# hyf015/egocentric-gaze-prediction

Measured on AMD Instinct MI355X. Metric: SP+AT train frames/sec/node (224x224, bs32/GPU), higher is better.
Workload: dtype f32 (every convolution -- forward, data gradient, weight gradient -- as f16 split-half MFMA, abs-max scaled operands, THREE products per MAC: 22 significant bits on both operands of every product; fp32 accumulate; everything else exact f32)

## Files before the change

### egocentric-gaze-prediction_amd/_lib.py

```python
from __future__ import annotations

import ctypes
import os
from ctypes import c_char_p, c_double, c_float, c_int, c_long, c_size_t, c_void_p

_HERE = os.path.dirname(os.path.abspath(__file__))
LIB_PATH = os.environ.get("EGAZE_HIP_LIB") or os.path.join(_HERE, "csrc", "libegaze_hip.so")

P = c_void_p
S = c_void_p

SIGNATURES = {
    "egz_version": (c_char_p, []),
    "egz_last_error": (c_char_p, []),
    "egz_mfma_probe": (c_int, [P, P, c_int, c_int, S]),
    "egz_u8_center_of_mass": (c_int, [P, c_int, c_int, c_int, P, P, P, S]),
    "egz_bilinear_up": (c_int, [P, P, c_int, c_int, c_int, c_int, c_int, c_long, S]),
    "egz_pack_w3x3_elems": (c_size_t, [c_int, c_int, c_int]),
    "egz_pack_w3x3_ups_fwd": (c_int, [P, P, c_int, c_int, S]),
    "egz_pack_w3x3_ups_dgrad": (c_int, [P, P, c_int, c_int, S]),
    "egz_conv3x3_ups_dgrad": (c_int, [P, P, P, c_int, c_int, c_int, c_int, c_int, c_int, S]),
    "egz_pack_w3x3_fwd": (c_int, [P, P, c_int, c_int, S]),
    "egz_pack_w3x3_dgrad": (c_int, [P, P, c_int, c_int, S]),
    "egz_conv3x3_stat_rows": (c_int, [c_int, c_int, c_int, c_int, c_int]),
# ... 66 lines not shown
    "egz_mse_bwd": (c_int, [P, P, P, P, c_long, c_int, S]),
    "egz_mse_fwd_grad": (c_int, [P, P, P, P, c_long, c_int, P, c_int, P, S]),
    "egz_gemm": (c_int, [P, P, P, P, c_int, c_int, c_int, c_long, c_long, c_long, c_long, c_long, c_int, S]),
    "egz_gemm_batched": (c_int, [P, P, P, c_int, c_int, c_int, c_int, c_long, c_long, c_long, c_long, c_long, c_int, S]),
    "egz_lstm_cell_fwd": (c_int, [P, P, P, P, P, c_int, c_int, S]),
    "egz_lstm_cell_bwd": (c_int, [P, P, P, P, P, P, P, c_int, c_int, S]),
    "egz_lstm_wave_fwd": (c_int, [P, P, P, P, P, P, P, P, P, P, P, c_int, c_int, c_int, c_int, S]),
    "egz_lstm_persist_sync_words": (c_int, []),
    "egz_lstm_persist_fwd": (c_int, [P, P, P, P, P, P, P, P, P, P, P, P, P, c_int, c_int, c_int, c_int, S]),
    "egz_lstm_persist_bwd": (c_int, [P, P, P, P, P, P, P, P, P, P, P, P, P, c_int, c_int, c_int, c_int, S]),
    "egz_lstm_wave_bwd": (c_int, [P, P, P, P, P, P, P, P, P, P, P, P, c_int, c_int, c_int, c_int, S]),
    "egz_lstm_b1_ws_bytes": (c_size_t, [c_int, c_int, c_int, c_int]),
    "egz_lstm_b1_fwd": (c_int, [P, c_int, P, P, P, P, P, P, P, P, c_int, c_int, c_int, S]),
    "egz_lstm_b1_bwd": (c_int, [P, P, c_int, P, P, P, P, P, P, P, P, P, P, c_int, c_int, c_int, P, c_size_t, S]),
    "egz_tanh_fwd": (c_int, [P, P, c_long, S]),
    "egz_tanh_bwd": (c_int, [P, P, P, c_long, S]),
    "egz_add": (c_int, [P, P, P, c_long, S]),
    "egz_cat2_planes": (c_int, [P, P, P, c_int, c_long, S]),
    "egz_u8_normalize": (c_int, [P, P, c_long, c_long, c_int, P, P, S]),
    "egz_crop_mean": (c_int, [P, P, P, c_int, c_int, c_int, c_int, c_int, c_int, S]),
    "egz_window_mean": (c_int, [P, P, P, c_int, c_int, c_int, c_int, S]),
    "egz_pixel_weighted_sum": (c_int, [P, P, P, c_int, c_int, c_int, S]),
    "egz_weighted_minmax": (c_int, [P, P, P, c_int, c_int, c_int, S]),
    "egz_aae_auc": (c_int, [P, P, c_int, c_int, c_int, P, c_int, c_double, P, S]),
    "egz_gaze_gt_maps": (c_int, [P, c_int, c_int, c_int, P, c_int, P, P, P, c_int, P, P, P, c_int, c_int, c_int, c_int,
                                 P, P, P, S]),
    "egz_resize_linear_u8": (c_int, [P, c_int, c_int, c_int, c_int, c_int, c_int, c_int, P, P, P, P, P, S]),
    "egz_heatmap_overlay": (c_int, [P, c_int, c_int, c_int, P, P, c_int, c_int, c_int, P, P, P, P, P, P, S]),
    "egz_cell_argmax_u8": (c_int, [P, c_int, c_int, c_int, c_int, P, S]),
    "egz_jpeg_decode_ws_bytes": (c_size_t, [c_int, c_int, c_int, c_int]),
    "egz_jpeg_decode": (c_int, [P, c_long, P, P, P, c_int, c_int, c_int, P, c_long, P, P, c_size_t, c_int, c_int, S]),
    "egz_adam_step": (c_int, [P, P, P, P, c_long, c_double, c_double, c_double, c_double, c_int, c_double, P, S]),
    "egz_adam_step_dev": (c_int, [P, P, P, P, c_long, c_double, c_double, c_double, c_double, P, c_double, P, S]),
}


class EgazeHipError(RuntimeError):
    """Raised when a C-ABI entry point returns a non-zero code (mirrors the reference's convention of
    plain Python exceptions: utils.generalException / RuntimeError, SURVEY.md 8b)."""


def _load():
    if not os.path.exists(LIB_PATH):
        raise ImportError(
            f"{LIB_PATH} is missing: the HIP extension is mandatory (no CPU fallback). "
            "Build it with `python __graft_entry__.py` or `csrc/build.sh`.")
    import torch
    lib = ctypes.CDLL(LIB_PATH)
    for name, (res, args) in SIGNATURES.items():
        try:
            fn = getattr(lib, name)
        except AttributeError as e:
            raise ImportError(f"{LIB_PATH} does not export {name}; rebuild the extension") from e
        fn.restype = res
        fn.argtypes = args
    return lib


LIB = _load()


def check(rc: int, what: str = ""):
    if rc != 0:
        msg = LIB.egz_last_error().decode(errors="replace")
        raise EgazeHipError(f"{what or 'egaze-hip'} failed (code {rc}): {msg}")

# ... 4 lines not shown
```

### egocentric-gaze-prediction_amd/csrc/adam.hip

```cpp
#include "egz_common.h"

namespace {
__global__ __launch_bounds__(256) void adam_kernel(float* __restrict__ p, const float* __restrict__ g, float* __restrict__ m,
                                                   float* __restrict__ v, long n, float omb1, float beta2, float omb2, float eps,
                                                   float step_size, float bc2_sqrt, float grad_scale,
                                                   unsigned int* __restrict__ nonfinite) {
#pragma clang fp contract(off)
    const long n4 = n >> 2;
    bool bad = false;
    for (long i = blockIdx.x * (long)blockDim.x + threadIdx.x; i < n4; i += (long)gridDim.x * blockDim.x) {
        f32x4 pv = reinterpret_cast<f32x4*>(p)[i];
        const f32x4 gv = reinterpret_cast<const f32x4*>(g)[i];
        f32x4 mv = reinterpret_cast<f32x4*>(m)[i];
        f32x4 vv = reinterpret_cast<f32x4*>(v)[i];
#pragma unroll
        for (int e = 0; e < 4; ++e) {
            const float ge = gv[e] * grad_scale;
            if (!(fabsf(ge) <= 3.402823466e38f)) { bad = true; continue; }
            mv[e] = mv[e] + omb1 * (ge - mv[e]);
            vv[e] = vv[e] * beta2 + omb2 * ge * ge;
            const float denom = sqrtf(vv[e]) / bc2_sqrt + eps;
            pv[e] = pv[e] - step_size * (mv[e] / denom);
        }
        reinterpret_cast<f32x4*>(p)[i] = pv;
        reinterpret_cast<f32x4*>(m)[i] = mv;
        reinterpret_cast<f32x4*>(v)[i] = vv;
    }
    const long t = n4 * 4 + blockIdx.x * (long)blockDim.x + threadIdx.x;
    if (t < n) {
        const float ge = g[t] * grad_scale;
        if (!(fabsf(ge) <= 3.402823466e38f)) bad = true;
        else {
            const float mm = m[t] + omb1 * (ge - m[t]);
// ... 19 lines not shown
    for (long i = blockIdx.x * (long)blockDim.x + threadIdx.x; i < n4; i += (long)gridDim.x * blockDim.x) {
        f32x4 pv = reinterpret_cast<f32x4*>(p)[i];
        const f32x4 gv = reinterpret_cast<const f32x4*>(g)[i];
        f32x4 mv = reinterpret_cast<f32x4*>(m)[i];
        f32x4 vv = reinterpret_cast<f32x4*>(v)[i];
#pragma unroll
        for (int e = 0; e < 4; ++e) {
            const float ge = gv[e] * grad_scale;
            if (!(fabsf(ge) <= 3.402823466e38f)) { bad = true; continue; }
            mv[e] = mv[e] + omb1 * (ge - mv[e]);
            vv[e] = vv[e] * b2 + omb2 * ge * ge;
            const float denom = sqrtf(vv[e]) / bc2_sqrt + eps;
            pv[e] = pv[e] - step_size * (mv[e] / denom);
        }
        reinterpret_cast<f32x4*>(p)[i] = pv;
        reinterpret_cast<f32x4*>(m)[i] = mv;
        reinterpret_cast<f32x4*>(v)[i] = vv;
    }
    const long tl = n4 * 4 + blockIdx.x * (long)blockDim.x + threadIdx.x;
    if (tl < n) {
        const float ge = g[tl] * grad_scale;
        if (!(fabsf(ge) <= 3.402823466e38f)) bad = true;
        else {
            const float mm = m[tl] + omb1 * (ge - m[tl]);
            const float vq = v[tl] * b2 + omb2 * ge * ge;
            m[tl] = mm;
            v[tl] = vq;
            p[tl] = p[tl] - step_size * (mm / (sqrtf(vq) / bc2_sqrt + eps));
        }
    }
    if (bad && nonfinite) atomicOr(nonfinite, 1u);
}
__global__ void adam_bump_kernel(int* step) { *step += 1; }
}

EGZ_API int egz_adam_step_dev(float* p, const float* g, float* m, float* v, long n, double lr, double beta1, double beta2,
                              double eps, int* step, double grad_scale, unsigned int* nonfinite, hipStream_t st) {
    EGZ_CHECK_ARG(p && g && m && v && step && n > 0, "egz_adam_step_dev: bad arguments");
    EGZ_CHECK_ARG(((uintptr_t)p % 16 == 0) && ((uintptr_t)g % 16 == 0) && ((uintptr_t)m % 16 == 0) && ((uintptr_t)v % 16 == 0),
                  "egz_adam_step_dev: buffers must be 16-byte aligned");
    long g4 = (n / 4 + 255) / 256;
    if (g4 < 1) g4 = 1;
    const int grid = (int)(g4 > 8192 ? 8192 : g4);
    hipLaunchKernelGGL(adam_dev_kernel, dim3(grid), dim3(256), 0, st, p, g, m, v, n, lr, beta1, beta2, (float)eps, step,
                       (float)grad_scale, nonfinite);
    EGZ_CHECK_LAUNCH("egz_adam_step_dev");
    hipLaunchKernelGGL(adam_bump_kernel, dim3(1), dim3(1), 0, st, step);
    EGZ_CHECK_LAUNCH("egz_adam_step_dev(bump)");
    return 0;
}

EGZ_API int egz_adam_step(float* p, const float* g, float* m, float* v, long n, double lr, double beta1, double beta2,
                          double eps, int step, double grad_scale, unsigned int* nonfinite, hipStream_t st) {
    EGZ_CHECK_ARG(p && g && m && v && n > 0 && step >= 1, "egz_adam_step: bad arguments");
    EGZ_CHECK_ARG(((uintptr_t)p % 16 == 0) && ((uintptr_t)g % 16 == 0) && ((uintptr_t)m % 16 == 0) && ((uintptr_t)v % 16 == 0),
                  "egz_adam_step: buffers must be 16-byte aligned");
    const double bc1 = 1.0 - pow(beta1, (double)step);
    const double bc2 = 1.0 - pow(beta2, (double)step);
    const float step_size = (float)(lr / bc1);
    const float bc2_sqrt = (float)sqrt(bc2);
    long g4 = (n / 4 + 255) / 256;
    if (g4 < 1) g4 = 1;
    const int grid = (int)(g4 > 8192 ? 8192 : g4);
    hipLaunchKernelGGL(adam_kernel, dim3(grid), dim3(256), 0, st, p, g, m, v, n,
                       (float)(1.0 - beta1), (float)beta2, (float)(1.0 - beta2), (float)eps, step_size, bc2_sqrt, (float)grad_scale, nonfinite);
    EGZ_CHECK_LAUNCH("egz_adam_step");
// ... 3 lines not shown
```

### egocentric-gaze-prediction_amd/csrc/conv3x3_igemm_x3s.hip

```cpp
#include "egz_common.h"
#include "x3_split.h"
#include <type_traits>



namespace {
using namespace x3;

enum { EPI_BIAS = 0, EPI_BIAS_RELU = 1, EPI_BIAS_STATS = 2, EPI_MASK_SUMS = 3, EPI_PARTIAL = 4, EPI_BNSUMS = 5 };
constexpr int XLD = 32;
constexpr int XBK = 32;
constexpr int HPITCH = 20;

template <int WM> struct Geo {
    static constexpr int WMM = WM;
    static constexpr int NWN = 4 / WM;
    static constexpr int NTHR = 64 * WMM * NWN;
    static constexpr int MR = (WM == 4) ? 2 : 4;
    static constexpr int RPW = 32 * MR;
    static constexpr int BM = RPW * WMM, BN = 32 * NWN;
    static constexpr int HSLOTS = (WM == 1) ? 256 : 384, HZERO = HSLOTS - 1;
    static constexpr int NABUF = (WM == 1) ? 2 : 1;
    static constexpr int PROWS = BM / 16;
    static constexpr int SPP = NTHR / 8;
    static constexpr int NJ = HSLOTS / SPP;
    static constexpr int OCC = (WM == 4) ? 3 : 2;
};

__device__ __forceinline__ void lds_barrier() { asm volatile("s_waitcnt lgkmcnt(0)\n\ts_barrier" ::: "memory"); }

enum { PLAIN = 0, UPSD = 1, UPSF = 2 };

__device__ __forceinline__ unsigned int ordered_bits(float f) {
    const unsigned int b = __float_as_uint(f);
// ... 530 lines not shown
            }
#pragma unroll
            for (int q = 0; q < SR; ++q) {
                const long srow = ((long)tile_m * G::WMM + wm) * SR + q;
                if (hl == 0 && nok && srow * 128 < M) {
                    stat[(srow * 2 + 0) * K + col] = s1b[q];
                    stat[(srow * 2 + 1) * K + col] = s2b[q];
                }
            }
        } else if (RPW == 128) {
            const long srow = (long)tile_m * G::WMM + wm;
            if (hl == 0 && nok && srow * 128 < M) {
                stat[(srow * 2 + 0) * K + col] = s1;
                stat[(srow * 2 + 1) * K + col] = s2;
            }
        } else {
            if (hl == 0) {
                sred[(wave * 2 + 0) * 32 + l31] = s1;
                sred[(wave * 2 + 1) * 32 + l31] = s2;
            }
            lds_barrier();
            const long srow = (long)tile_m * (BM / 128) + (wm >> 1);
            if ((wm & 1) == 0 && hl == 0 && nok && srow * 128 < M) {
                stat[(srow * 2 + 0) * K + col] = s1 + sred[((wave + NWN) * 2 + 0) * 32 + l31];
                stat[(srow * 2 + 1) * K + col] = s2 + sred[((wave + NWN) * 2 + 1) * 32 + l31];
            }
        }
    }
#ifdef EGZ_TILE_LOOP
    }
#endif
}

__device__ __forceinline__ float weff9s(const float* __restrict__ w9, int py, int a, int px, int b) {
    const int rlo = (py == 0) ? (a == 0 ? 0 : 1) : (a == 0 ? 0 : 2), rhi = (py == 0) ? (a == 0 ? 0 : 2) : (a == 0 ? 1 : 2);
    const int slo = (px == 0) ? (b == 0 ? 0 : 1) : (b == 0 ? 0 : 2), shi = (px == 0) ? (b == 0 ? 0 : 2) : (b == 0 ? 1 : 2);
    float s = 0.f;
    for (int r = rlo; r <= rhi; ++r)
        for (int q = slo; q <= shi; ++q) s += w9[r * 3 + q];
    return s;
}

__device__ __forceinline__ float frag_value9(const float* w9, int kind, int si) {
    if (kind == 4) return w9[si];
    if (kind == 5) return w9[8 - si];
    if (kind == 7) return weff9s(w9, (si >> 2) >> 1, (si & 3) >> 1, (si >> 2) & 1, si & 1);
    const int img = si >> 2, tap = si & 3;
    const int oy = 2 * (tap >> 1) - (img >> 1), ox = 2 * (tap & 1) - (img & 1);
    return weff9s(w9, (oy == -1 || oy == 1) ? 1 : 0, (oy <= 0) ? 1 : 0, (ox == -1 || ox == 1) ? 1 : 0, (ox <= 0) ? 1 : 0);
}

template <typename T, int KIND>
__device__ __forceinline__ void frag_pack_pair(const float* __restrict__ w, unsigned short* __restrict__ wq, int C, int K,
                                               int Np, int Rp, float scale, long j) {
    constexpr int NS = (KIND >= 6) ? 16 : 9;
    const int nt32 = Np >> 5, ncb = Rp / XBK;
    const int e = (int)(j & 7), lane = (int)((j >> 3) & 63), ks = (int)((j >> 9) & 1);
    const long r2 = j >> 10;
    const int ntile = (int)(r2 % nt32), cblk = (int)(r2 / nt32);
    const int col = ntile * 32 + (lane & 31), k = cblk * XBK + ks * 16 + (lane >> 5) * 8 + e;
    float w9[9];
    const bool fwd = (KIND == 4 || KIND == 7);
    const bool ok = fwd ? (col < K && k < C) : (col < C && k < K);
    const float* src = w + (fwd ? ((long)col * C + k) : ((long)k * C + col)) * 9;
#pragma unroll
    for (int t = 0; t < 9; ++t) w9[t] = ok ? src[t] : 0.f;
#pragma unroll
    for (int si = 0; si < NS; ++si) {
        const long s = (KIND == 7) ? (long)(si >> 2) * (ncb * 4) + cblk * 4 + (si & 3) : (long)cblk * NS + si;
        const long r = s * nt32 + ntile;
        unsigned short h, l;
        Half<T>::split(frag_value9(w9, KIND, si) * scale, h, l);
        const long base = ((r * 2 + ks) * 2) * 512 + lane * 8 + e;
        wq[base] = h;
        wq[base + 512] = l;
    }
}
template <typename T>
__device__ __forceinline__ void frag_pack_pair_k(const float* __restrict__ w, unsigned short* __restrict__ wq, int C, int K,
                                                 int kind, int Np, int Rp, float scale, long j) {
    if (kind == 4) frag_pack_pair<T, 4>(w, wq, C, K, Np, Rp, scale, j);
    else if (kind == 5) frag_pack_pair<T, 5>(w, wq, C, K, Np, Rp, scale, j);
    else if (kind == 6) frag_pack_pair<T, 6>(w, wq, C, K, Np, Rp, scale, j);
    else frag_pack_pair<T, 7>(w, wq, C, K, Np, Rp, scale, j);
}

template <typename T>
__global__ __launch_bounds__(256) void pack_split_frag_kernel(const float* __restrict__ w, unsigned short* __restrict__ wq,
                                                             int C, int K, int kind, int Np, int Rp, float scale) {
    const long n = (long)Np * Rp;
    for (long j = blockIdx.x * (long)blockDim.x + threadIdx.x; j < n; j += (long)gridDim.x * blockDim.x)
        frag_pack_pair_k<T>(w, wq, C, K, kind, Np, Rp, scale, j);
}


constexpr int PT_LD = 289;
template <typename T>
__device__ __forceinline__ void pack_frag_tile(const float* __restrict__ w, unsigned short* __restrict__ wq, int C, int K,
                                               int kind, float scale, int tile, float* __restrict__ sw) {
    const int Cp = (C + 31) & ~31, Kp = (K + 31) & ~31;
    const int ncbc = Cp >> 5;
    const int kb = tile / ncbc, cb = tile - kb * ncbc;
    const int tid = threadIdx.x;
    if (C % 32 == 0 && (reinterpret_cast<unsigned long long>(w) & 15) == 0) {
        for (int idx = tid; idx < 32 * 72; idx += 256) {
            const int i = idx / 72, q = idx - i * 72;
            const int k = kb * 32 + i;
            f32x4 v = f32x4{0.f, 0.f, 0.f, 0.f};
            if (k < K) v = *reinterpret_cast<const f32x4*>(w + ((long)k * C + cb * 32) * 9 + q * 4);
            float* d = sw + i * PT_LD + q * 4;
            d[0] = v[0]; d[1] = v[1]; d[2] = v[2]; d[3] = v[3];
        }
    } else {
        for (int idx = tid; idx < 32 * 288; idx += 256) {
            const int i = idx / 288, q = idx - i * 288;
            const int k = kb * 32 + i, c = cb * 32 + q / 9;
            sw[i * PT_LD + q] = (k < K && c < C) ? w[(long)k * C * 9 + cb * 288 + q] : 0.f;
        }
    }
    __syncthreads();
    const bool fwd = (kind == 4 || kind == 7);
    const int NS = (kind >= 6) ? 16 : 9;
    const int nt32 = (fwd ? Kp : Cp) >> 5, ncb = (fwd ? Cp : Kp) >> 5;
    const int ntile = fwd ? kb : cb, cblk = fwd ? cb : kb;
    for (int it = tid; it < NS * 128; it += 256) {
        const int lane = it & 63, ks = (it >> 6) & 1, si = it >> 7;
        const int col = lane & 31, kk0 = ks * 16 + (lane >> 5) * 8;
        const float* p = fwd ? sw + col * PT_LD + kk0 * 9 : sw + kk0 * PT_LD + col * 9;
        const int estep = fwd ? 9 : PT_LD;
        unsigned short h[8], l[8];
#pragma unroll
        for (int e = 0; e < 8; ++e) {
            const float* pe = p + e * estep;
            float v;
            if (kind == 4) v = pe[si];
            else if (kind == 5) v = pe[8 - si];
            else {
                float w9[9];
#pragma unroll
                for (int t = 0; t < 9; ++t) w9[t] = pe[t];
                v = frag_value9(w9, kind, si);
            }
            Half<T>::split(v * scale, h[e], l[e]);
        }
        const long s = (kind == 7) ? (long)(si >> 2) * (ncb * 4) + cblk * 4 + (si & 3) : (long)cblk * NS + si;
        const long r = s * nt32 + ntile;
        const long base = ((r * 2 + ks) * 2) * 512 + lane * 8;
        u32x4 hv, lv;
#pragma unroll
        for (int e = 0; e < 4; ++e) {
            hv[e] = (unsigned)h[2 * e] | ((unsigned)h[2 * e + 1] << 16);
            lv[e] = (unsigned)l[2 * e] | ((unsigned)l[2 * e + 1] << 16);
        }
        *reinterpret_cast<u32x4*>(wq + base) = hv;
        *reinterpret_cast<u32x4*>(wq + base + 512) = lv;
    }
}

__global__ __launch_bounds__(256) void pack_frag_batch_kernel(const long long* __restrict__ table, int n) {
    __shared__ float sw[32 * PT_LD];
    const int b = (int)blockIdx.x;
    int lo = 0, hi = n - 1;
    while (lo < hi) {
        const int mid = (lo + hi + 1) >> 1;
        if (table[mid * 8 + 6] <= b) lo = mid; else hi = mid - 1;
    }
    const long long* d = table + lo * 8;
    const float* w = reinterpret_cast<const float*>(d[0]);
    unsigned short* wq = reinterpret_cast<unsigned short*>(d[1]);
    const int C = (int)d[2], K = (int)d[3], kind = (int)d[4], tile = b - (int)d[6];
    if (d[5] == 1) pack_frag_tile<_Float16>(w, wq, C, K, kind, F16_WSCALE, tile, sw);
    else pack_frag_tile<__bf16>(w, wq, C, K, kind, 1.f, tile, sw);
}


template <typename T, int EPI, bool BNIN>
__global__ __launch_bounds__(256, 1) void conv3x3_x3p_narrow_kernel(
    const float* __restrict__ x, const unsigned short* __restrict__ wq, const float* __restrict__ bias,
    float* __restrict__ y, double* __restrict__ stat, int B, int H, int W, int C, int K, float out_scale, int total,
    const unsigned int* __restrict__ a_absmax, const float* __restrict__ bn_y, const float* __restrict__ bn_coef,
    float* __restrict__ mm_out) {
    using G = Geo<4>;
    constexpr int BM = G::BM, HSLOTS = G::HSLOTS, NJ = G::NJ, SPP = G::SPP, MR = G::MR, RPW = G::RPW;
    constexpr int APL = HSLOTS * XLD, ABUF = 2 * APL;
    static_assert(BM == 256 && MR == 2 && RPW == 64 && G::PROWS == 16, "16 x 16 patch, 64 rows per wave");
    __shared__ __attribute__((aligned(16))) unsigned short Ah[2 * ABUF];
    __shared__ double sred[4 * 2 * 32];

    const float a_scale = absmax_scale(a_absmax);
// ... 665 lines not shown
```

### egocentric-gaze-prediction_amd/hipops.py

```python
from __future__ import annotations

import weakref
from typing import Optional, Tuple

import torch

from ._lib import LIB as _RAW_LIB, check

EPI_BIAS, EPI_BIAS_RELU, EPI_BIAS_STATS = 0, 1, 2
import os as _os


class _Profiler:

    def __init__(self):
        self.enabled = False
        self.events = {}
        self.flops = {}

    def start(self):
        self.events, self.flops, self.enabled = {}, {}, True

    def stop(self):
        self.enabled = False
# ... 170 lines not shown


def packed_weight(w: torch.Tensor, kind: str, dtype: int = 0) -> torch.Tensor:
    _req(w, "weight")
    K, C = w.shape[0], w.shape[1]
    key = (_uid(w), kind, dtype)
    tag = _tag(w)
    hit = _PACKED.get(key)
    if hit is not None and hit[0] == tag:
        _USED.add(key)
        return hit[1]
    fname, ekind, kidx = _PACK_FN[kind]
    buf = hit[1] if hit is not None else torch.empty(LIB.egz_pack_w3x3_elems(C, K, ekind), dtype=torch.float32,
                                                     device=w.device)
    if kidx >= 4:
        if not dtype:
            raise RuntimeError("fragment-ordered packings exist for the split-half dtypes only")
        check(LIB.egz_pack_w3x3_split_frag(w.data_ptr(), buf.data_ptr(), C, K, kidx, dtype, _stream()),
              "egz_pack_w3x3_split_frag")
    elif dtype:
        check(LIB.egz_pack_w3x3_split(w.data_ptr(), buf.data_ptr(), C, K, kidx, dtype, _stream()), "egz_pack_w3x3_split")
    else:
        check(getattr(LIB, fname)(w.data_ptr(), buf.data_ptr(), C, K, _stream()), fname)
    _PACKED[key] = (tag, buf, weakref.ref(w))
    _USED.add(key)
    return buf


BATCH_REPACK = True
_BATCH_TABLES = {}
_BATCH_PINNED = set()


def refresh_packings(params, force: bool = False) -> int:
    if not BATCH_REPACK or not (_USED or force):
        return 0
    ids = {getattr(p, "_egz_uid", None) for p in params}
    todo = []
    for key in sorted(k for k in (_PACKED if force else _USED) if k[0] in ids and k[2] and _PACK_FN[k[1]][2] >= 4):
        hit = _PACKED.get(key)
        w = hit[2]() if hit is not None else None
        if w is None:
            _USED.discard(key)
            continue
        if force or hit[0] != _tag(w):
            todo.append((key, w, hit[1]))
    if not todo:
        return 0
    sig = tuple((key, w.data_ptr(), buf.data_ptr()) for key, w, buf in todo)
    ent = _BATCH_TABLES.get(sig)
    capturing = torch.cuda.is_current_stream_capturing()
    if ent is None and capturing:
        for key, w, buf in todo:
            check(LIB.egz_pack_w3x3_split_frag(w.data_ptr(), buf.data_ptr(), w.shape[1], w.shape[0], _PACK_FN[key[1]][2], key[2],
                                               _stream()), "egz_pack_w3x3_split_frag")
    else:
        if ent is None:
            rows, nb = [], 0
            for key, w, buf in todo:
                K, C = w.shape[0], w.shape[1]
                rows.append([w.data_ptr(), buf.data_ptr(), C, K, _PACK_FN[key[1]][2], key[2], nb, 0])
                nb += LIB.egz_pack_w3x3_frag_blocks(C, K)
            if len(_BATCH_TABLES) > 64:
                for k_ in [k_ for k_ in _BATCH_TABLES if k_ not in _BATCH_PINNED]:
                    del _BATCH_TABLES[k_]
            ent = (torch.tensor(rows, dtype=torch.int64).to(todo[0][1].device), nb)
            _BATCH_TABLES[sig] = ent
        if capturing:
            _BATCH_PINNED.add(sig)
        check(LIB.egz_pack_w3x3_frag_batch(ent[0].data_ptr(), len(todo), ent[1], _stream()), "egz_pack_w3x3_frag_batch")
    for key, w, buf in todo:
        _PACKED[key] = (_tag(w), buf, weakref.ref(w))
        _USED.discard(key)
    return len(todo)


def repack_stale(params) -> int:
    ids = {getattr(p, "_egz_uid", None) for p in params}
    n = 0
    for key in [k for k in _PACKED if k[0] in ids]:
        hit = _PACKED.get(key)
        w = hit[2]() if hit is not None else None
        if w is not None and hit[0] != _tag(w):
            packed_weight(w, key[1], key[2])
            n += 1
    return n


class GradSink:
    __slots__ = ("buf", "owner", "gen_written", "hooks")

    def __init__(self, buf, owner):
        self.buf, self.owner, self.gen_written, self.hooks = buf, owner, -1, []


def grad_sink(param, wanted: bool = True) -> Optional[torch.Tensor]:
    if not wanted:
        return None
    sk = getattr(param, "_egz_sink", None)
    if sk is None or not DIRECT_GRADS:
        return None
    gen = sk.owner.zero_gen
    if sk.gen_written == gen:
        return None
    sk.gen_written = gen
    return sk.buf

# ... 1623 lines not shown
```

### egocentric-gaze-prediction_amd/optim.py

```python
from __future__ import annotations

from typing import Iterable, List

import os

import torch

from . import hipops as H
from . import streams




class FusedAdam:
    def __init__(self, params, lr: float = 1e-3, betas=(0.9, 0.999), eps: float = 1e-8):
        params = list(params)
        if params and isinstance(params[0], dict):
            if len(params) != 1:
                raise NotImplementedError("the reference uses a single parameter group")
            group = params[0]
            lr = group.get("lr", lr)
            params = list(group["params"])
        self.params: List[torch.nn.Parameter] = [p for p in params if p.requires_grad]
        if not self.params:
# ... 38 lines not shown
    def check_finite(self, reset: bool = True) -> None:
        if int(self.nonfinite.item()):
            if reset:
                self.nonfinite.zero_()
            raise FloatingPointError("FusedAdam: a step since the last check saw NaN / inf gradient elements and skipped them "
                                     "(parameters untouched there); the backward pass that produced them is broken -- e.g. a "
                                     "persistent-LSTM hand-off that timed out (hipops.lstm_persist_check)")

    def note_replays(self, n: int = 1):
        self.step_count += n

    def zero_grad(self, set_to_none: bool = False, all_overwritten: bool = False):
        from . import functions as _F
        _F._JOIN_QUEUED[0] = False
        if all_overwritten:
            pass
        else:
            H.fill_zero(self.flat_g)
        self.zero_gen += 1
        for p, o in zip(self.params, self.offsets):
            if p.grad is None or p.grad.data_ptr() != self.flat_g.data_ptr() + 4 * o:
                p.grad = self.flat_g[o:o + p.numel()].view(p.shape)

    @torch.no_grad()
    def step(self):
        from . import functions as _F
        _F._JOIN_QUEUED[0] = False
        for hook in self.pre_step_hooks:
            hook()
        capturing = torch.cuda.is_current_stream_capturing()
        if not capturing:
            streams.join_all_into_current()
        self.step_count += 1
        if self.capturable:
            H.adam_step_dev(self.flat_p, self.flat_g, self.flat_m, self.flat_v, self.lr, self.betas[0], self.betas[1],
                            self.eps, self.step_dev, self.grad_scale, nonfinite=self.nonfinite)
        else:
            if capturing:
                raise RuntimeError("FusedAdam.step() inside a hipGraph capture needs set_capturable(True)")
            H.adam_step(self.flat_p, self.flat_g, self.flat_m, self.flat_v, self.lr, self.betas[0], self.betas[1],
                        self.eps, self.step_count, self.grad_scale, nonfinite=self.nonfinite)
        H.touch_params(self.params)
        H.refresh_packings(self.params)

    @property
    def param_groups(self):
        return [dict(self.defaults, lr=self.lr, maximize=False, foreach=None, capturable=False, differentiable=False,
                     fused=None, decoupled_weight_decay=False, params=list(range(len(self.params))))]

    def state_dict(self):
        state = {}
        if self.step_count > 0:
            for i, (p, o) in enumerate(zip(self.params, self.offsets)):
                n = p.numel()
                state[i] = {"step": torch.tensor(float(self.step_count)),
                            "exp_avg": self.flat_m[o:o + n].view(p.shape).clone(),
                            "exp_avg_sq": self.flat_v[o:o + n].view(p.shape).clone()}
        return {"state": state, "param_groups": self.param_groups}

    def load_state_dict(self, sd):
        groups = sd.get("param_groups", [])
        if groups and "params" in groups[0] and len(groups[0]["params"]) != len(self.params):
            raise ValueError("loaded state dict contains a parameter group that doesn't match the size of "
                             "optimizer's group")
        if groups:
            self.lr = groups[0].get("lr", self.lr)
            self.betas = tuple(groups[0].get("betas", self.betas))
            self.eps = groups[0].get("eps", self.eps)
        with torch.no_grad():
            for i, (p, o) in enumerate(zip(self.params, self.offsets)):
                st = sd["state"].get(i)
                if st is None:
                    continue
                n = p.numel()
                self.flat_m[o:o + n].copy_(st["exp_avg"].reshape(-1))
# ... 8 lines not shown
```

### include/egaze_hip.h

```cpp
#ifndef EGAZE_HIP_H
#define EGAZE_HIP_H

#include <stddef.h>

#ifdef __cplusplus
extern "C" {
#endif

typedef struct ihipStream_t* hipStream_t;

const char* egz_version(void);
const char* egz_last_error(void);

size_t egz_pack_w3x3_elems(int C, int K, int kind );
int egz_pack_w3x3_fwd(const float* w, float* wp, int C, int K, hipStream_t stream);
int egz_pack_w3x3_dgrad(const float* w, float* wp, int C, int K, hipStream_t stream);
int egz_pack_w3x3_ups_fwd(const float* w, float* wp, int C, int K, hipStream_t stream);
int egz_pack_w3x3_ups_dgrad(const float* w, float* wp, int C, int K, hipStream_t stream);
int egz_conv3x3_stat_rows(int B, int H, int W, int K, int flags);
int egz_conv3x3_fwd(const float* x, const float* wp, const float* bias, float* y, double* stat_partial, int B, int H,
                    int W, int C, int K, int flags, hipStream_t stream);
int egz_conv3x3_ups_dgrad(const float* dy, const float* wp, float* dx, int B, int H, int W, int C, int K, int flags,
                          hipStream_t stream);
int egz_pack_w3x3_split(const float* w, void* wp, int C, int K, int kind, int dtype, hipStream_t stream);
// ... 115 lines not shown
                     long sak, long sbk, long sbn, long ldc, int flags, hipStream_t stream);
int egz_lstm_cell_fwd(const float* gates, const float* c_prev, float* h_out, float* c_out, float* act, int B, int Hd,
                      hipStream_t stream);
int egz_lstm_cell_bwd(const float* act, const float* c, const float* c_prev, const float* dh, const float* dc_in,
                      float* dgates, float* dc_prev, int B, int Hd, hipStream_t stream);
int egz_lstm_wave_fwd(const float* gx0, const float* const* w_ih, const float* const* w_hh, const float* const* bsum,
                      const float* h0, const float* c0, float* hs, float* cs, float* acts, float* hn, float* cn, int L, int T,
                      int B, int H, hipStream_t stream);
int egz_lstm_persist_sync_words(void);
int egz_lstm_persist_fwd(const float* gx0, const float* const* w_ih, const float* const* w_hh, const float* const* b_ih,
                         const float* const* b_hh, const float* h0, const float* c0, float* hs, float* cs, float* acts, float* hn,
                         float* cn, unsigned int* sync, int L, int T, int B, int H, hipStream_t stream);
int egz_lstm_wave_bwd(const float* dh_top, const float* dhn, const float* dcn, const float* acts, const float* cs,
                      const float* c0, const float* const* w_hh_t, const float* const* w_ih_t, float* dgates, float* dh0,
                      float* dc0, float* dhin, int L, int T, int B, int H, hipStream_t stream);
int egz_lstm_persist_bwd(const float* dh_top, const float* dhn, const float* dcn, const float* acts, const float* cs,
                         const float* c0, const float* const* w_hh, const float* const* w_ih, float* dgates, float* dh0,
                         float* dc0, float* const* db, unsigned int* sync, int L, int T, int B, int H, hipStream_t stream);
size_t egz_lstm_b1_ws_bytes(int L, int C, int H, int N);
int egz_lstm_b1_fwd(const void* const* params, int L, const float* inp, const float* h0, const float* c0, float* xt,
                    float* acts, float* hn, float* cn, float* out, int C, int H, int N, hipStream_t stream);
int egz_lstm_b1_bwd(const void* const* params, void* const* grads, int L, const float* dout, const float* dhn,
                    const float* dcn, const float* xt, const float* acts, const float* h0, const float* c0,
                    const float* hn, const float* cn, const float* out, int C, int H, int N, void* workspace,
                    size_t ws_bytes, hipStream_t stream);
int egz_tanh_fwd(const float* x, float* y, long n, hipStream_t stream);
int egz_tanh_bwd(const float* y, const float* dy, float* dx, long n, hipStream_t stream);
int egz_add(const float* a, const float* b, float* out, long n, hipStream_t stream);

int egz_adam_step(float* p, const float* g, float* m, float* v, long n, double lr, double beta1, double beta2,
                  double eps, int step, double grad_scale, unsigned int* nonfinite, hipStream_t stream);
int egz_adam_step_dev(float* p, const float* g, float* m, float* v, long n, double lr, double beta1, double beta2,
                      double eps, int* step, double grad_scale, unsigned int* nonfinite, hipStream_t stream);

int egz_aae_auc(const float* out, const float* gt, int B, int H, int W, const double* gw, int R, double dist,
                double* res, hipStream_t stream);

int egz_gaze_gt_maps(const int* pos, int N, int H, int W, const double* gw, int R, const int* xofs, const int* xsi,
                     const float* xalpha, int nx, const int* yofs, const int* ysi, const float* yalpha, int ny, int mode,
                     int oh, int ow, unsigned char* out_u8, double* out_f64, double* out_full, hipStream_t stream);

int egz_resize_linear_u8(const unsigned char* src, int N, int C, int sh, int sw, int dh, int dw, int interleaved,
                         const int* xofs, const short* xalpha, const int* yofs, const short* yalpha, unsigned char* dst,
                         hipStream_t stream);
int egz_heatmap_overlay(const unsigned char* maps, int M, int h, int w, const int* frame_index, const unsigned char* frames,
                        int F, int H, int W, const unsigned char* lut, const int* xofs, const short* xalpha, const int* yofs,
                        const short* yalpha, unsigned char* out, hipStream_t stream);
int egz_cell_argmax_u8(const unsigned char* gt, int N, int H, int W, int cell, int* out, hipStream_t stream);

size_t egz_jpeg_decode_ws_bytes(int N, int H, int W, int n3);
int egz_jpeg_decode(const unsigned char* data, long data_len, const long* offsets, const int* channels, const long* planes,
                    int N, int H, int W, unsigned char* out, long out_planes, int* status, void* ws, size_t ws_bytes,
                    int n3, int stages, hipStream_t stream);

int egz_cat2_planes(const float* f, const float* g, float* out, int B, long HW, hipStream_t stream);
int egz_u8_normalize(const unsigned char* src, float* dst, long n, long plane, int C, const float* mean,
                     const float* std, hipStream_t stream);
int egz_crop_mean(const float* feat, const int* gp, float* out, int B, int H, int W, int C, int size, int cell,
                  hipStream_t stream);
int egz_window_mean(const float* feat, const int* win, float* out, int B, int H, int W, int C, hipStream_t stream);
int egz_pixel_weighted_sum(const float* feat, const float* wmap, float* out, int B, int HW, int C, hipStream_t stream);
int egz_weighted_minmax(const float* feat, const float* w, float* out, int B, int HW, int C, hipStream_t stream);

int egz_u8_center_of_mass(const float* map, int B, int H, int W, double* com, int* gp, unsigned char* q8, hipStream_t stream);
int egz_bilinear_up(const float* src, float* dst, int B, int h, int w, int scale, int align_corners, long dst_bstride,
                    hipStream_t stream);
// ... 8 lines not shown
```

Baseline: 1112.

## Fuse Adam update with split-half weight fragment repacking in one kernel

Adds a fused kernel in which each 3x3 conv weight tile is updated by Adam, staged in shared memory, and immediately emitted as packed f16/bf16 split-half MFMA fragments. Non-conv parameter ranges are handled by chunked blocks in the same launch. This removes the separate repack pass that re-read the updated weights and saves a kernel launch, at the cost of host-side table building and a more complex optimizer path. The fragment emission code is moved into a shared header.

```diff
diff --git a/egocentric-gaze-prediction_amd/_lib.py b/egocentric-gaze-prediction_amd/_lib.py
--- a/egocentric-gaze-prediction_amd/_lib.py
+++ b/egocentric-gaze-prediction_amd/_lib.py
@@ -122,6 +122,9 @@
     "egz_jpeg_decode": (c_int, [P, c_long, P, P, P, c_int, c_int, c_int, P, c_long, P, P, c_size_t, c_int, c_int, S]),
     "egz_adam_step": (c_int, [P, P, P, P, c_long, c_double, c_double, c_double, c_double, c_int, c_double, P, S]),
     "egz_adam_step_dev": (c_int, [P, P, P, P, c_long, c_double, c_double, c_double, c_double, P, c_double, P, S]),
+    "egz_adam_pack_step": (c_int, [P, P, P, P, c_long, P, c_int, c_int, P, c_int, c_double, c_double, c_double, c_double, c_int, P,
+                                   c_double, P, S]),
+    "egz_adam_pack_chunk": (c_int, []),
 }
 
 
diff --git a/egocentric-gaze-prediction_amd/csrc/adam.hip b/egocentric-gaze-prediction_amd/csrc/adam.hip
--- a/egocentric-gaze-prediction_amd/csrc/adam.hip
+++ b/egocentric-gaze-prediction_amd/csrc/adam.hip
@@ -1,4 +1,5 @@
 #include "egz_common.h"
+#include "pack_frag.h"
 
 namespace {
 __global__ __launch_bounds__(256) void adam_kernel(float* __restrict__ p, const float* __restrict__ g, float* __restrict__ m,
@@ -84,6 +85,171 @@
     if (bad && nonfinite) atomicOr(nonfinite, 1u);
 }
 __global__ void adam_bump_kernel(int* step) { *step += 1; }
+
+constexpr int ADAM_CHUNK = 4096;
+constexpr int AP_ROW = 16;
+
+struct AdamScalars {
+    float omb1, beta2, omb2, eps, step_size, bc2_sqrt, grad_scale;
+};
+
+__device__ __forceinline__ bool adam_elem(float& p, const float g, float& m, float& v, const AdamScalars& a) {
+#pragma clang fp contract(off)
+    const float ge = g * a.grad_scale;
+    if (!(fabsf(ge) <= 3.402823466e38f)) return false;
+    m = m + a.omb1 * (ge - m);
+    v = v * a.beta2 + a.omb2 * ge * ge;
+    const float denom = sqrtf(v) / a.bc2_sqrt + a.eps;
+    p = p - a.step_size * (m / denom);
+    return true;
+}
+
+__device__ __forceinline__ bool adam_quad(f32x4& p, const f32x4 g, f32x4& m, f32x4& v, const AdamScalars& a) {
+    bool ok = true;
+#pragma unroll
+    for (int e = 0; e < 4; ++e) {
+        float pe = p[e], me = m[e], ve = v[e];
+        ok &= adam_elem(pe, g[e], me, ve, a);
+        p[e] = pe; m[e] = me; v[e] = ve;
+    }
+    return ok;
+}
+
+template <bool DEV>
+__global__ __launch_bounds__(256) void adam_pack_kernel(float* __restrict__ p, const float* __restrict__ g, float* __restrict__ m,
+                                                        float* __restrict__ v, long n, const long long* __restrict__ rows,
+                                                        int n_rows, int tile_blocks, const long long* __restrict__ chunks,
+                                                        AdamScalars a, double lr, double beta1, double beta2d,
+                                                        const int* __restrict__ step, unsigned int* __restrict__ nonfinite) {
+#pragma clang fp contract(off)
+    __shared__ float sw[32 * x3::PT_LD];
+    if (DEV) {
+        const double t = (double)(*static_cast<const volatile int*>(step) + 1);
+        a.omb1 = (float)(1.0 - beta1);
+        a.beta2 = (float)beta2d;
+        a.omb2 = (float)(1.0 - beta2d);
+        a.step_size = (float)(lr / (1.0 - pow(beta1, t)));
+        a.bc2_sqrt = (float)sqrt(1.0 - pow(beta2d, t));
+    }
+    const int tid = threadIdx.x;
+    const int b = (int)blockIdx.x;
+    bool bad = false;
+    if (b >= tile_blocks) {
+        long lo = chunks[(long)(b - tile_blocks) * 2], hi = chunks[(long)(b - tile_blocks) * 2 + 1];
+        lo = lo < 0 ? 0 : lo;
+        hi = hi > n ? n : hi;
+        const long va = (lo + 3) & ~3L, vb = hi & ~3L;
+        for (long i = (va >> 2) + tid; i < (vb >> 2); i += 256) {
+            f32x4 pv = reinterpret_cast<f32x4*>(p)[i];
+            const f32x4 gv = reinterpret_cast<const f32x4*>(g)[i];
+            f32x4 mv = reinterpret_cast<f32x4*>(m)[i];
+            f32x4 vv = reinterpret_cast<f32x4*>(v)[i];
+            bad |= !adam_quad(pv, gv, mv, vv, a);
+            reinterpret_cast<f32x4*>(p)[i] = pv;
+            reinterpret_cast<f32x4*>(m)[i] = mv;
+            reinterpret_cast<f32x4*>(v)[i] = vv;
+        }
+        long t = -1;
+        if (va > vb) { if (lo + tid < hi) t = lo + tid; }
+        else if (tid < 4) { if (lo + tid < va) t = lo + tid; }
+        else if (tid < 8) { if (vb + (tid - 4) < hi) t = vb + (tid - 4); }
+        if (t >= 0) {
+            float pe = p[t], me = m[t], ve = v[t];
+            if (adam_elem(pe, g[t], me, ve, a)) { p[t] = pe; m[t] = me; v[t] = ve; }
+            else bad = true;
+        }
+        if (bad && nonfinite) atomicOr(nonfinite, 1u);
+        return;
+    }
+    int rl = 0, rh = n_rows - 1;
+    while (rl < rh) {
+        const int mid = (rl + rh + 1) >> 1;
+        if (rows[mid * AP_ROW + 3] <= b) rl = mid; else rh = mid - 1;
+    }
+    const long long* d = rows + rl * AP_ROW;
+    const long off = (long)d[0];
+    const int C = (int)d[1], K = (int)d[2], tile = b - (int)d[3], npack = (int)d[4];
+    if (off < 0 || off + (long)K * C * 9 > n) return;
+    const int ncbc = (C + 31) >> 5;
+    const int kb = tile / ncbc, cb = tile - kb * ncbc;
+    if (C % 32 == 0 && (off & 3) == 0) {
+#pragma unroll 3
+        for (int idx = tid; idx < 32 * 72; idx += 256) {
+            const int i = idx / 72, q = idx - i * 72;
+            const int k = kb * 32 + i;
+            f32x4 pv = f32x4{0.f, 0.f, 0.f, 0.f};
+            if (k < K) {
+                const long o = off + ((long)k * C + cb * 32) * 9 + q * 4;
+                pv = *reinterpret_cast<const f32x4*>(p + o);
+                const f32x4 gv = *reinterpret_cast<const f32x4*>(g + o);
+                f32x4 mv = *reinterpret_cast<const f32x4*>(m + o);
+                f32x4 vv = *reinterpret_cast<const f32x4*>(v + o);
+                bad |= !adam_quad(pv, gv, mv, vv, a);
+                *reinterpret_cast<f32x4*>(p + o) = pv;
+                *reinterpret_cast<f32x4*>(m + o) = mv;
+                *reinterpret_cast<f32x4*>(v + o) = vv;
+            }
+            float* s = sw + i * x3::PT_LD + q * 4;
+            s[0] = pv[0]; s[1] = pv[1]; s[2] = pv[2]; s[3] = pv[3];
+        }
+    } else {
+        for (int idx = tid; idx < 32 * 288; idx += 256) {
+            const int i = idx / 288, q = idx - i * 288;
+            const int k = kb * 32 + i, c = cb * 32 + q / 9;
+            float pe = 0.f;
+            if (k < K && c < C) {
+                const long o = off + (long)k * C * 9 + cb * 288 + q;
+                pe = p[o];
+                float me = m[o], ve = v[o];
+                if (adam_elem(pe, g[o], me, ve, a)) { p[o] = pe; m[o] = me; v[o] = ve; }
+                else bad = true;
+            }
+            sw[i * x3::PT_LD + q] = pe;
+        }
+    }
+    if (bad && nonfinite) atomicOr(nonfinite, 1u);
+    __syncthreads();
+    for (int j = 0; j < npack && j < 4; ++j) {
+        unsigned short* wq = reinterpret_cast<unsigned short*>(d[8 + 2 * j]);
+        const int kind = (int)(d[9 + 2 * j] & 0xff), dtype = (int)(d[9 + 2 * j] >> 8);
+        if (dtype == 1) x3::pack_frag_emit<_Float16>(sw, wq, C, K, kind, x3::F16_WSCALE, tile);
+        else x3::pack_frag_emit<__bf16>(sw, wq, C, K, kind, 1.f, tile);
+    }
+}
+}
+
+EGZ_API int egz_adam_pack_chunk(void) { return ADAM_CHUNK; }
+
+EGZ_API int egz_adam_pack_step(float* p, const float* g, float* m, float* v, long n, const long long* rows, int n_rows,
+                               int tile_blocks, const long long* chunks, int n_chunks, double lr, double beta1, double beta2,
+                               double eps, int step, int* step_dev, double grad_scale, unsigned int* nonfinite, hipStream_t st) {
+    EGZ_CHECK_ARG(p && g && m && v && n > 0 && rows && n_rows > 0 && tile_blocks > 0 && n_chunks >= 0 && (chunks || n_chunks == 0)
+                  && (step_dev || step >= 1), "egz_adam_pack_step: bad arguments");
+    EGZ_CHECK_ARG(((uintptr_t)p % 16 == 0) && ((uintptr_t)g % 16 == 0) && ((uintptr_t)m % 16 == 0) && ((uintptr_t)v % 16 == 0),
+                  "egz_adam_pack_step: buffers must be 16-byte aligned");
+    EGZ_CHECK_ARG((long)tile_blocks + n_chunks < (1L << 31), "egz_adam_pack_step: too many blocks");
+    AdamScalars a;
+    a.omb1 = (float)(1.0 - beta1);
+    a.beta2 = (float)beta2;
+    a.omb2 = (float)(1.0 - beta2);
+    a.eps = (float)eps;
+    a.grad_scale = (float)grad_scale;
+    a.step_size = a.bc2_sqrt = 0.f;
+    const dim3 grid(tile_blocks + n_chunks);
+    if (step_dev) {
+        hipLaunchKernelGGL(adam_pack_kernel<true>, grid, dim3(256), 0, st, p, g, m, v, n, rows, n_rows, tile_blocks, chunks, a,
+                           lr, beta1, beta2, (const int*)step_dev, nonfinite);
+        EGZ_CHECK_LAUNCH("egz_adam_pack_step");
+        hipLaunchKernelGGL(adam_bump_kernel, dim3(1), dim3(1), 0, st, step_dev);
+        EGZ_CHECK_LAUNCH("egz_adam_pack_step(bump)");
+    } else {
+        a.step_size = (float)(lr / (1.0 - pow(beta1, (double)step)));
+        a.bc2_sqrt = (float)sqrt(1.0 - pow(beta2, (double)step));
+        hipLaunchKernelGGL(adam_pack_kernel<false>, grid, dim3(256), 0, st, p, g, m, v, n, rows, n_rows, tile_blocks, chunks, a,
+                           lr, beta1, beta2, (const int*)nullptr, nonfinite);
+        EGZ_CHECK_LAUNCH("egz_adam_pack_step");
+    }
+    return 0;
 }
 
 EGZ_API int egz_adam_step_dev(float* p, const float* g, float* m, float* v, long n, double lr, double beta1, double beta2,
diff --git a/egocentric-gaze-prediction_amd/csrc/conv3x3_igemm_x3s.hip b/egocentric-gaze-prediction_amd/csrc/conv3x3_igemm_x3s.hip
--- a/egocentric-gaze-prediction_amd/csrc/conv3x3_igemm_x3s.hip
+++ b/egocentric-gaze-prediction_amd/csrc/conv3x3_igemm_x3s.hip
@@ -1,5 +1,6 @@
 #include "egz_common.h"
 #include "x3_split.h"
+#include "pack_frag.h"
 #include <type_traits>
 
 
@@ -596,23 +597,6 @@
 #endif
 }
 
-__device__ __forceinline__ float weff9s(const float* __restrict__ w9, int py, int a, int px, int b) {
-    const int rlo = (py == 0) ? (a == 0 ? 0 : 1) : (a == 0 ? 0 : 2), rhi = (py == 0) ? (a == 0 ? 0 : 2) : (a == 0 ? 1 : 2);
-    const int slo = (px == 0) ? (b == 0 ? 0 : 1) : (b == 0 ? 0 : 2), shi = (px == 0) ? (b == 0 ? 0 : 2) : (b == 0 ? 1 : 2);
-    float s = 0.f;
-    for (int r = rlo; r <= rhi; ++r)
-        for (int q = slo; q <= shi; ++q) s += w9[r * 3 + q];
-    return s;
-}
-
-__device__ __forceinline__ float frag_value9(const float* w9, int kind, int si) {
-    if (kind == 4) return w9[si];
-    if (kind == 5) return w9[8 - si];
-    if (kind == 7) return weff9s(w9, (si >> 2) >> 1, (si & 3) >> 1, (si >> 2) & 1, si & 1);
-    const int img = si >> 2, tap = si & 3;
-    const int oy = 2 * (tap >> 1) - (img >> 1), ox = 2 * (tap & 1) - (img & 1);
-    return weff9s(w9, (oy == -1 || oy == 1) ? 1 : 0, (oy <= 0) ? 1 : 0, (ox == -1 || ox == 1) ? 1 : 0, (ox <= 0) ? 1 : 0);
-}
 
 template <typename T, int KIND>
 __device__ __forceinline__ void frag_pack_pair(const float* __restrict__ w, unsigned short* __restrict__ wq, int C, int K,
@@ -658,12 +642,10 @@
 }
 
 
-constexpr int PT_LD = 289;
 template <typename T>
 __device__ __forceinline__ void pack_frag_tile(const float* __restrict__ w, unsigned short* __restrict__ wq, int C, int K,
                                                int kind, float scale, int tile, float* __restrict__ sw) {
-    const int Cp = (C + 31) & ~31, Kp = (K + 31) & ~31;
-    const int ncbc = Cp >> 5;
+    const int ncbc = (C + 31) >> 5;
     const int kb = tile / ncbc, cb = tile - kb * ncbc;
     const int tid = threadIdx.x;
     if (C % 32 == 0 && (reinterpret_cast<unsigned long long>(w) & 15) == 0) {
@@ -683,42 +665,7 @@
         }
     }
     __syncthreads();
-    const bool fwd = (kind == 4 || kind == 7);
-    const int NS = (kind >= 6) ? 16 : 9;
-    const int nt32 = (fwd ? Kp : Cp) >> 5, ncb = (fwd ? Cp : Kp) >> 5;
-    const int ntile = fwd ? kb : cb, cblk = fwd ? cb : kb;
-    for (int it = tid; it < NS * 128; it += 256) {
-        const int lane = it & 63, ks = (it >> 6) & 1, si = it >> 7;
-        const int col = lane & 31, kk0 = ks * 16 + (lane >> 5) * 8;
-        const float* p = fwd ? sw + col * PT_LD + kk0 * 9 : sw + kk0 * PT_LD + col * 9;
-        const int estep = fwd ? 9 : PT_LD;
-        unsigned short h[8], l[8];
-#pragma unroll
-        for (int e = 0; e < 8; ++e) {
-            const float* pe = p + e * estep;
-            float v;
-            if (kind == 4) v = pe[si];
-            else if (kind == 5) v = pe[8 - si];
-            else {
-                float w9[9];
-#pragma unroll
-                for (int t = 0; t < 9; ++t) w9[t] = pe[t];
-                v = frag_value9(w9, kind, si);
-            }
-            Half<T>::split(v * scale, h[e], l[e]);
-        }
-        const long s = (kind == 7) ? (long)(si >> 2) * (ncb * 4) + cblk * 4 + (si & 3) : (long)cblk * NS + si;
-        const long r = s * nt32 + ntile;
-        const long base = ((r * 2 + ks) * 2) * 512 + lane * 8;
-        u32x4 hv, lv;
-#pragma unroll
-        for (int e = 0; e < 4; ++e) {
-            hv[e] = (unsigned)h[2 * e] | ((unsigned)h[2 * e + 1] << 16);
-            lv[e] = (unsigned)l[2 * e] | ((unsigned)l[2 * e + 1] << 16);
-        }
-        *reinterpret_cast<u32x4*>(wq + base) = hv;
-        *reinterpret_cast<u32x4*>(wq + base + 512) = lv;
-    }
+    pack_frag_emit<T>(sw, wq, C, K, kind, scale, tile);
 }
 
 __global__ __launch_bounds__(256) void pack_frag_batch_kernel(const long long* __restrict__ table, int n) {
diff --git a/egocentric-gaze-prediction_amd/csrc/pack_frag.h b/egocentric-gaze-prediction_amd/csrc/pack_frag.h
--- /dev/null
+++ b/egocentric-gaze-prediction_amd/csrc/pack_frag.h
@@ -0,0 +1,71 @@
+#pragma once
+#include "x3_split.h"
+
+namespace x3 {
+
+__device__ __forceinline__ float weff9s(const float* __restrict__ w9, int py, int a, int px, int b) {
+    const int rlo = (py == 0) ? (a == 0 ? 0 : 1) : (a == 0 ? 0 : 2), rhi = (py == 0) ? (a == 0 ? 0 : 2) : (a == 0 ? 1 : 2);
+    const int slo = (px == 0) ? (b == 0 ? 0 : 1) : (b == 0 ? 0 : 2), shi = (px == 0) ? (b == 0 ? 0 : 2) : (b == 0 ? 1 : 2);
+    float s = 0.f;
+    for (int r = rlo; r <= rhi; ++r)
+        for (int q = slo; q <= shi; ++q) s += w9[r * 3 + q];
+    return s;
+}
+
+__device__ __forceinline__ float frag_value9(const float* w9, int kind, int si) {
+    if (kind == 4) return w9[si];
+    if (kind == 5) return w9[8 - si];
+    if (kind == 7) return weff9s(w9, (si >> 2) >> 1, (si & 3) >> 1, (si >> 2) & 1, si & 1);
+    const int img = si >> 2, tap = si & 3;
+    const int oy = 2 * (tap >> 1) - (img >> 1), ox = 2 * (tap & 1) - (img & 1);
+    return weff9s(w9, (oy == -1 || oy == 1) ? 1 : 0, (oy <= 0) ? 1 : 0, (ox == -1 || ox == 1) ? 1 : 0, (ox <= 0) ? 1 : 0);
+}
+
+constexpr int PT_LD = 289;
+
+template <typename T>
+__device__ __forceinline__ void pack_frag_emit(const float* __restrict__ sw, unsigned short* __restrict__ wq, int C, int K,
+                                               int kind, float scale, int tile) {
+    const int Cp = (C + 31) & ~31, Kp = (K + 31) & ~31;
+    const int ncbc = Cp >> 5;
+    const int kb = tile / ncbc, cb = tile - kb * ncbc;
+    const int tid = threadIdx.x;
+    const bool fwd = (kind == 4 || kind == 7);
+    const int NS = (kind >= 6) ? 16 : 9;
+    const int nt32 = (fwd ? Kp : Cp) >> 5, ncb = (fwd ? Cp : Kp) >> 5;
+    const int ntile = fwd ? kb : cb, cblk = fwd ? cb : kb;
+    for (int it = tid; it < NS * 128; it += 256) {
+        const int lane = it & 63, ks = (it >> 6) & 1, si = it >> 7;
+        const int col = lane & 31, kk0 = ks * 16 + (lane >> 5) * 8;
+        const float* p = fwd ? sw + col * PT_LD + kk0 * 9 : sw + kk0 * PT_LD + col * 9;
+        const int estep = fwd ? 9 : PT_LD;
+        unsigned short h[8], l[8];
+#pragma unroll
+        for (int e = 0; e < 8; ++e) {
+            const float* pe = p + e * estep;
+            float v;
+            if (kind == 4) v = pe[si];
+            else if (kind == 5) v = pe[8 - si];
+            else {
+                float w9[9];
+#pragma unroll
+                for (int t = 0; t < 9; ++t) w9[t] = pe[t];
+                v = frag_value9(w9, kind, si);
+            }
+            Half<T>::split(v * scale, h[e], l[e]);
+        }
+        const long s = (kind == 7) ? (long)(si >> 2) * (ncb * 4) + cblk * 4 + (si & 3) : (long)cblk * NS + si;
+        const long r = s * nt32 + ntile;
+        const long base = ((r * 2 + ks) * 2) * 512 + lane * 8;
+        u32x4 hv, lv;
+#pragma unroll
+        for (int e = 0; e < 4; ++e) {
+            hv[e] = (unsigned)h[2 * e] | ((unsigned)h[2 * e + 1] << 16);
+            lv[e] = (unsigned)l[2 * e] | ((unsigned)l[2 * e + 1] << 16);
+        }
+        *reinterpret_cast<u32x4*>(wq + base) = hv;
+        *reinterpret_cast<u32x4*>(wq + base + 512) = lv;
+    }
+}
+
+}
diff --git a/egocentric-gaze-prediction_amd/hipops.py b/egocentric-gaze-prediction_amd/hipops.py
--- a/egocentric-gaze-prediction_amd/hipops.py
+++ b/egocentric-gaze-prediction_amd/hipops.py
@@ -226,9 +226,7 @@
 _BATCH_PINNED = set()
 
 
-def refresh_packings(params, force: bool = False) -> int:
-    if not BATCH_REPACK or not (_USED or force):
-        return 0
+def _stale_frag_packings(params, force: bool = False):
     ids = {getattr(p, "_egz_uid", None) for p in params}
     todo = []
     for key in sorted(k for k in (_PACKED if force else _USED) if k[0] in ids and k[2] and _PACK_FN[k[1]][2] >= 4):
@@ -239,6 +237,13 @@
             continue
         if force or hit[0] != _tag(w):
             todo.append((key, w, hit[1]))
+    return todo
+
+
+def refresh_packings(params, force: bool = False) -> int:
+    if not BATCH_REPACK or not (_USED or force):
+        return 0
+    todo = _stale_frag_packings(params, force)
     if not todo:
         return 0
     sig = tuple((key, w.data_ptr(), buf.data_ptr()) for key, w, buf in todo)
@@ -267,6 +272,72 @@
         _PACKED[key] = (_tag(w), buf, weakref.ref(w))
         _USED.discard(key)
     return len(todo)
+
+
+FUSED_ADAM_PACK = True
+
+
+def adam_pack_step(params, p, g, m, v, lr, beta1, beta2, eps, step, step_dev=None, grad_scale=1.0, nonfinite=None) -> int:
+    if not (FUSED_ADAM_PACK and BATCH_REPACK and PRECISION == "split" and _USED):
+        return -1
+    n, base = p.numel(), p.data_ptr()
+    groups = {}
+    for key, w, buf in _stale_frag_packings(params):
+        off = w.data_ptr() - base
+        K, C = w.shape[0], w.shape[1]
+        if (w.dim() == 4 and w.shape[2:] == (3, 3) and w.is_contiguous() and w.dtype == torch.float32 and off % 4 == 0
+                and 0 <= off // 4 and off // 4 + K * C * 9 <= n and buf.data_ptr() % 16 == 0):
+            ent = groups.setdefault(off // 4, (w, []))
+            if len(ent[1]) < 4:
+                ent[1].append((key, buf))
+    if not groups:
+        return -1
+    order = sorted(groups)
+    sig = ("adam", base, n) + tuple((key, o, buf.data_ptr()) for o in order for key, buf in groups[o][1])
+    ent = _BATCH_TABLES.get(sig)
+    capturing = torch.cuda.is_current_stream_capturing()
+    if ent is None:
+        if capturing:
+            return -1
+        rows, ranges, nb, end = [], [], 0, 0
+        for o in order:
+            w, packs = groups[o]
+            K, C = w.shape[0], w.shape[1]
+            if o < end:
+                raise RuntimeError("adam_pack_step: overlapping parameters in the flat buffer")
+            if o > end:
+                ranges.append((end, o))
+            end = o + K * C * 9
+            row = [o, C, K, nb, len(packs), 0, 0, 0] + [0] * 8
+            for j, (key, buf) in enumerate(packs):
+                row[8 + 2 * j], row[9 + 2 * j] = buf.data_ptr(), _PACK_FN[key[1]][2] | (key[2] << 8)
+            rows.append(row)
+            nb += LIB.egz_pack_w3x3_frag_blocks(C, K)
+        if end < n:
+            ranges.append((end, n))
+        ch = LIB.egz_adam_pack_chunk()
+        chunks = [(a, min(a + ch, hi)) for lo, hi in ranges for a in range(lo, hi, ch)]
+        if len(_BATCH_TABLES) > 64:
+            for k_ in [k_ for k_ in _BATCH_TABLES if k_ not in _BATCH_PINNED]:
+                del _BATCH_TABLES[k_]
+        dev = p.device
+        ent = (torch.tensor(rows, dtype=torch.int64).to(dev), nb,
+               torch.tensor(chunks, dtype=torch.int64).reshape(-1, 2).to(dev), len(chunks))
+        _BATCH_TABLES[sig] = ent
+    if capturing:
+        _BATCH_PINNED.add(sig)
+    check(LIB.egz_adam_pack_step(p.data_ptr(), g.data_ptr(), m.data_ptr(), v.data_ptr(), n, ent[0].data_ptr(), len(order), ent[1],
+                                 ent[2].data_ptr() if ent[3] else None, ent[3], lr, beta1, beta2, eps,
+                                 0 if step_dev is not None else int(step), _p(step_dev), grad_scale, _p(nonfinite), _stream()),
+          "egz_adam_pack_step")
+    done = 0
+    for o in order:
+        w, packs = groups[o]
+        for key, buf in packs:
+            _PACKED[key] = (_tag(w), buf, weakref.ref(w))
+            _USED.discard(key)
+            done += 1
+    return done
 
 
 def repack_stale(params) -> int:
diff --git a/egocentric-gaze-prediction_amd/optim.py b/egocentric-gaze-prediction_amd/optim.py
--- a/egocentric-gaze-prediction_amd/optim.py
+++ b/egocentric-gaze-prediction_amd/optim.py
@@ -94,15 +94,18 @@
         if not capturing:
             streams.join_all_into_current()
         self.step_count += 1
-        if self.capturable:
-            H.adam_step_dev(self.flat_p, self.flat_g, self.flat_m, self.flat_v, self.lr, self.betas[0], self.betas[1],
-                            self.eps, self.step_dev, self.grad_scale, nonfinite=self.nonfinite)
-        else:
-            if capturing:
-                raise RuntimeError("FusedAdam.step() inside a hipGraph capture needs set_capturable(True)")
-            H.adam_step(self.flat_p, self.flat_g, self.flat_m, self.flat_v, self.lr, self.betas[0], self.betas[1],
-                        self.eps, self.step_count, self.grad_scale, nonfinite=self.nonfinite)
+        if capturing and not self.capturable:
+            raise RuntimeError("FusedAdam.step() inside a hipGraph capture needs set_capturable(True)")
         H.touch_params(self.params)
+        if H.adam_pack_step(self.params, self.flat_p, self.flat_g, self.flat_m, self.flat_v, self.lr, self.betas[0],
+                            self.betas[1], self.eps, self.step_count, self.step_dev if self.capturable else None,
+                            self.grad_scale, nonfinite=self.nonfinite) < 0:
+            if self.capturable:
+                H.adam_step_dev(self.flat_p, self.flat_g, self.flat_m, self.flat_v, self.lr, self.betas[0], self.betas[1],
+                                self.eps, self.step_dev, self.grad_scale, nonfinite=self.nonfinite)
+            else:
+                H.adam_step(self.flat_p, self.flat_g, self.flat_m, self.flat_v, self.lr, self.betas[0], self.betas[1],
+                            self.eps, self.step_count, self.grad_scale, nonfinite=self.nonfinite)
         H.refresh_packings(self.params)
 
     @property
diff --git a/include/egaze_hip.h b/include/egaze_hip.h
--- a/include/egaze_hip.h
+++ b/include/egaze_hip.h
@@ -171,6 +171,10 @@
                   double eps, int step, double grad_scale, unsigned int* nonfinite, hipStream_t stream);
 int egz_adam_step_dev(float* p, const float* g, float* m, float* v, long n, double lr, double beta1, double beta2,
                       double eps, int* step, double grad_scale, unsigned int* nonfinite, hipStream_t stream);
+int egz_adam_pack_step(float* p, const float* g, float* m, float* v, long n, const long long* rows, int n_rows,
+                       int tile_blocks, const long long* chunks, int n_chunks, double lr, double beta1, double beta2,
+                       double eps, int step, int* step_dev, double grad_scale, unsigned int* nonfinite, hipStream_t stream);
+int egz_adam_pack_chunk(void);
 
 int egz_aae_auc(const float* out, const float* gt, int B, int H, int W, const double* gw, int R, double dist,
                 double* res, hipStream_t stream);
```

After: 1115, median of 6. About the same (+0.3%).
